# mpkuse/cerebro

Measured on AMD Instinct MI355X. Metric: loop-queries/sec (ticks of 3 descriptors vs 4096-D x 1M DB), higher is better.
Workload: dtype f64

## Files before the change

cerebro_amd/capi.py:

```python
from __future__ import annotations

import ctypes as C
import os
import sys
from pathlib import Path

import numpy as np

_HERE = Path(__file__).resolve().parent
PRODUCT_LIB_PATH = _HERE / "lib" / "libcerebro_hip.so"
HOOKS_LIB_PATH = _HERE / "lib" / "hooks" / "libcerebro_hip.so"


def _lib_path() -> Path:
    override = os.environ.get("CHIP_LIB")
    if override:
        if os.environ.get("CHIP_ALLOW_LIB_OVERRIDE") == "1":
            return Path(override).resolve()
        sys.stderr.write(f"[cerebro_amd] CHIP_LIB={override} IGNORED: set CHIP_ALLOW_LIB_OVERRIDE=1 to load another build of the library\n")
    return PRODUCT_LIB_PATH


LIB_PATH = _lib_path()

# ... 164 lines not shown
    "chip_loop_tick_enqueue": (C.c_int, [_P, C.c_int64, C.POINTER(DotParams), C.c_int32]),
    "chip_loop_tick_collect": (C.c_int, [_P, C.c_int32, C.POINTER(TickResult)]),
    "chip_loop_last_l": (C.c_int64, [_P]),
    "chip_loop_reset": (None, [_P]),
    "chip_scan_local": (C.c_int, [_P, C.c_int64, C.POINTER(DotParams), C.c_int32, _P, C.POINTER(C.c_int32)]),
    "chip_merge_decide": (C.c_int, [_P, C.c_int64, C.POINTER(DotParams), _P, C.c_int32, C.c_int32, C.POINTER(TickResult)]),
    "chip_merge_decide_enqueue": (C.c_int, [_P, C.c_int64, C.POINTER(DotParams), _P, C.c_int32, C.c_int32, C.c_int32]),
    "chip_debug_merge_lists": (C.c_int, [_P, C.c_int32, _P, C.c_int32, C.c_int32, C.c_int32, _P, C.c_int64, C.POINTER(DotParams),
                                         C.POINTER(TickResult)]),
    "chip_ransac_params_default": (None, [C.POINTER(RansacParams)]),
    "chip_pnp_ransac": (C.c_int, [_P, _P, _P, C.c_int32, C.POINTER(RansacParams), _P, C.POINTER(C.c_float), _P,
                                  C.POINTER(RansacSummary)]),
    "chip_pnp_ransac_batch": (C.c_int, [_P, C.c_int32, _P, _P, _P, C.POINTER(RansacParams), _P, _P, _P, _P, _P]),
    "chip_icp_params_default": (None, [C.POINTER(RansacParams)]),
    "chip_icp_ransac": (C.c_int, [_P, _P, _P, C.c_int32, C.POINTER(RansacParams), _P, C.POINTER(C.c_float), _P,
                                  C.POINTER(RansacSummary)]),
    "chip_icp_ransac_enqueue": (C.c_int, [_P, _P, _P, C.c_int32, C.POINTER(RansacParams)]),
    "chip_icp_ransac_collect": (C.c_int, [_P, _P, C.POINTER(C.c_float), _P, C.POINTER(RansacSummary)]),
    "chip_build_has_icp_batch": (C.c_int, []),
    "chip_icp_ransac_batch": (C.c_int, [_P, C.c_int32, _P, _P, _P, C.POINTER(RansacParams), _P, _P, _P, _P, _P]),
    "chip_debug_ransac_record": (C.c_int, [_P, C.c_int32, C.c_int32, C.POINTER(RansacShape), _P, _P, _P, _P, _P, _P, _P]),
    "chip_debug_pnp_stage": (C.c_int, [_P, C.c_int32, _P, _P, _P]),
    "chip_debug_pnp_keep_stage": (C.c_int, [_P, C.c_int32]),
    "chip_build_has_match": (C.c_int, []),
    "chip_build_has_tick_coalesce": (C.c_int, []),
    "chip_debug_coalesce_stats": (C.c_int, [_P, C.POINTER(C.c_int64), C.POINTER(C.c_int64)]),
    "chip_debug_coalesce_force": (C.c_int, [_P, C.c_int32]),
    "chip_debug_coalesce_decide": (C.c_int, [C.c_int32, C.c_int32, C.c_int32]),
    "chip_debug_last_scan": (C.c_int, [_P, C.POINTER(ScanLaunch)]),
    "chip_debug_scan_plan": (C.c_int, [C.c_int32, C.c_int32, C.c_int32, C.c_int32, C.c_int64, C.c_int32, C.c_int32, C.POINTER(ScanLaunch)]),
    "chip_debug_multi_plan": (C.c_int, [C.c_int32, C.c_int32, C.c_int32, C.c_int32, C.c_int32, C.POINTER(ScanLaunch)]),
    "chip_debug_prefilter_plan": (C.c_int, [C.c_int32, C.c_int32, C.c_int32, C.c_int32, C.POINTER(ScanLaunch)]),
    "chip_debug_prefilter_stats": (C.c_int, [_P, C.POINTER(C.c_int64), C.POINTER(C.c_int64), C.POINTER(C.c_int64)]),
    "chip_orb_match": (C.c_int, [_P, _P, C.c_int32, _P, C.c_int32, _P, _P]),
    "chip_gms_filter": (C.c_int, [_P, _P, C.c_int32, C.c_int32, C.c_int32, _P, C.c_int32, C.c_int32, C.c_int32, _P, _P, C.c_int32, _P,
                                  C.POINTER(C.c_int32)]),
    "chip_match_pair": (C.c_int, [_P, C.POINTER(MatchFrame), C.POINTER(MatchFrame), _P, C.POINTER(MatchSummary)]),
    "chip_match_read_sets": (C.c_int, [_P, C.POINTER(MatchSetsOut)]),
    "chip_pnp_ransac_matched": (C.c_int, [_P, C.c_int32, C.POINTER(RansacParams), _P, C.POINTER(C.c_float), _P, C.POINTER(RansacSummary)]),
    "chip_icp_ransac_matched": (C.c_int, [_P, C.POINTER(RansacParams), _P, C.POINTER(C.c_float), _P, C.POINTER(RansacSummary)]),
    "chip_build_has_gms_modes": (C.c_int, []),
    "chip_gms_filter_modes": (C.c_int, [_P, _P, C.c_int32, C.c_int32, C.c_int32, _P, C.c_int32, C.c_int32, C.c_int32, _P, _P, C.c_int32,
                                        C.c_uint32, _P, C.POINTER(C.c_int32), C.POINTER(GmsChoice)]),
    "chip_match_batch_modes": (C.c_int, [_P, C.POINTER(MatchFrame), C.POINTER(MatchFrame), C.c_int32, _P, C.c_uint32, C.POINTER(MatchSummary),
                                         C.POINTER(GmsChoice)]),
    "chip_match_batch_stored_modes": (C.c_int, [_P, C.c_int64, _P, C.c_int32, _P, C.c_uint32, C.POINTER(MatchSummary), C.POINTER(GmsChoice)]),
    "chip_build_has_match_batch": (C.c_int, []),
    "chip_match_batch": (C.c_int, [_P, C.POINTER(MatchFrame), C.POINTER(MatchFrame), C.c_int32, _P, C.POINTER(MatchSummary)]),
    "chip_match_select": (C.c_int, [_P, C.c_int32]),
    "chip_match_batch_read_matches": (C.c_int, [_P, C.c_int32, _P, _P]),
    "chip_pnp_ransac_matched_batch": (C.c_int, [_P, C.c_int32, _P, _P, C.POINTER(RansacParams), _P, _P, _P, _P, _P, _P]),
    "chip_icp_ransac_matched_batch_enqueue": (C.c_int, [_P, C.c_int32, _P, C.POINTER(RansacParams), _P, _P]),
    "chip_icp_ransac_matched_batch_collect": (C.c_int, [_P, _P, _P, _P, _P]),
    "chip_icp_ransac_matched_batch": (C.c_int, [_P, C.c_int32, _P, C.POINTER(RansacParams), _P, _P, _P, _P, _P, _P]),
    "chip_build_has_frame_store": (C.c_int, []),
    "chip_frame_store_reserve": (C.c_int, [_P, C.c_int32, C.c_int32]),
    "chip_frame_store_info": (C.c_int, [_P, C.POINTER(C.c_int32), C.POINTER(C.c_int32), C.POINTER(C.c_int32)]),
    "chip_frame_put": (C.c_int, [_P, C.c_int64, C.POINTER(MatchFrame)]),
    "chip_frame_drop": (C.c_int, [_P, C.c_int64]),
    "chip_frame_read": (C.c_int, [_P, C.c_int64, C.POINTER(C.c_int32), C.POINTER(C.c_int32), C.POINTER(C.c_int32), _P, _P, _P]),
    "chip_match_batch_stored": (C.c_int, [_P, C.c_int64, _P, C.c_int32, _P, C.POINTER(MatchSummary)]),
    "chip_build_has_match_pairs": (C.c_int, []),
    "chip_match_pairs_stored": (C.c_int, [_P, _P, _P, C.c_int32, _P, C.c_uint32, C.POINTER(MatchSummary), C.POINTER(GmsChoice)]),
    "chip_get_info": (C.c_int, [_P, C.POINTER(Info)]),
    "chip_profile_enable": (C.c_int, [_P, C.c_int32]),
    "chip_profile_reset": (C.c_int, [_P]),
# ... 271 lines not shown
        return r

    def resident_pause(self):
        self._chk(self.lib.chip_resident_pause(self.h), "chip_resident_pause")

    def resident_resume(self):
        self._chk(self.lib.chip_resident_resume(self.h), "chip_resident_resume")

    def loop_tick_enqueue(self, l: int, slot: int, params: DotParams | None = None):
        p = params or default_dot_params()
        self._chk(self.lib.chip_loop_tick_enqueue(self.h, l, C.byref(p), slot), "chip_loop_tick_enqueue")

    def loop_tick_collect(self, slot: int) -> TickResult:
        r = TickResult()
        self._chk(self.lib.chip_loop_tick_collect(self.h, slot, C.byref(r)), "chip_loop_tick_collect")
        return r

    def loop_reset(self):
        self.lib.chip_loop_reset(self.h)

    def last_l(self) -> int:
        return int(self.lib.chip_loop_last_l(self.h))

    def coalesce_stats(self) -> tuple[int, int]:
        passes, ticks = C.c_int64(), C.c_int64()
        self._chk(self.lib.chip_debug_coalesce_stats(self.h, C.byref(passes), C.byref(ticks)), "chip_debug_coalesce_stats")
        return passes.value, ticks.value

    def prefilter_stats(self) -> tuple[int, int, int]:
        passes, ticks, unc = C.c_int64(), C.c_int64(), C.c_int64()
        self._chk(self.lib.chip_debug_prefilter_stats(self.h, C.byref(passes), C.byref(ticks), C.byref(unc)), "chip_debug_prefilter_stats")
        return passes.value, ticks.value, unc.value

    def coalesce_force(self, on: bool):
        self._chk(self.lib.chip_debug_coalesce_force(self.h, 1 if on else 0), "chip_debug_coalesce_force")

    def last_scan(self) -> dict:
        out = ScanLaunch()
        self._chk(self.lib.chip_debug_last_scan(self.h, C.byref(out)), "chip_debug_last_scan")
        return out.as_dict()

    def scan_local(self, l: int, dev_out_ptr: int, topk: int = CHIP_DEFAULT_TOPK, params: DotParams | None = None) -> int:
        p = params or default_dot_params()
        status = C.c_int32()
        self._chk(self.lib.chip_scan_local(self.h, l, C.byref(p), topk, C.c_void_p(dev_out_ptr), C.byref(status)),
                  "chip_scan_local")
        return status.value

    def merge_decide(self, l: int, dev_gathered_ptr: int, n_lists: int, topk: int = CHIP_DEFAULT_TOPK,
                     params: DotParams | None = None) -> TickResult:
        p = params or default_dot_params()
        r = TickResult()
        self._chk(self.lib.chip_merge_decide(self.h, l, C.byref(p), C.c_void_p(dev_gathered_ptr), n_lists, topk,
                                             C.byref(r)), "chip_merge_decide")
        return r

    def merge_decide_enqueue(self, l: int, dev_gathered_ptr: int, n_lists: int, slot: int, topk: int = CHIP_DEFAULT_TOPK,
                             params: DotParams | None = None):
        p = params or default_dot_params()
        self._chk(self.lib.chip_merge_decide_enqueue(self.h, l, C.byref(p), C.c_void_p(dev_gathered_ptr), n_lists, topk, slot),
                  "chip_merge_decide_enqueue")

    def debug_merge_lists(self, form: int, scores: np.ndarray, idx: np.ndarray, l: int = 0, params: DotParams | None = None,
                          record: bool = False):
        scores = np.ascontiguousarray(scores, dtype=np.float64)
        idx = np.ascontiguousarray(idx, dtype=np.int64)
# ... 399 lines not shown
```

cerebro_amd/csrc/chip_api.hip:

```cpp
#include "chip_internal.h"
#include <cmath>
#include <cstdlib>
#include <cstring>
#include <memory>
#include <new>

using namespace chip;

extern "C" {

const char *chip_strerror(int status)
{
    switch (status) {
        case CHIP_OK: return "ok";
        case CHIP_ERR_INVALID_ARG: return "invalid argument";
        case CHIP_ERR_NO_DEVICE: return "no usable HIP device";
        case CHIP_ERR_HIP: return "HIP runtime error (see chip_last_hip_error)";
        case CHIP_ERR_OOM: return "out of device memory";
        case CHIP_ERR_NOT_F32: return "descriptor value not exactly representable as float32";
        case CHIP_ERR_NONFINITE: return "NaN/Inf in descriptor";
        case CHIP_ERR_RANGE: return "index / length out of range";
        case CHIP_ERR_UNSUPPORTED: return "unsupported configuration";
        case CHIP_ERR_TOO_FEW_POINTS: return "fewer than 20 correspondences";
        case CHIP_ERR_BUSY: return "async slot busy or empty";
// ... 176 lines not shown
    int rc = c->seg_table_dev.alloc(c, kMaxSegs);
    if (rc == CHIP_OK) rc = configure_storage(c, elem);
    if (rc != CHIP_OK) return rc;
    c->stage_bytes = 64ull << 20;
    if (c->stage_bytes < (size_t)c->D * 8 * 64) c->stage_bytes = (size_t)c->D * 8 * 64;
    rc = c->stage_dev.alloc(c, c->stage_bytes);
    if (rc == CHIP_OK) rc = c->flags_dev.alloc(c, 1);
    if (rc == CHIP_OK) rc = c->flags_host.alloc(c, 1);
    if (rc == CHIP_OK) rc = c->norm2_dev.alloc(c, 1);
    if (rc == CHIP_OK) rc = c->norm2_host.alloc(c, 1);
    if (rc != CHIP_OK) return rc;
    CHIP_HIP(c, hipMemset(c->norm2_dev, 0, sizeof(unsigned long long)));
    *c->norm2_host.host() = 0;

    scan_read_knobs(c);
    CHIP_HIP(c, hipStreamCreateWithFlags(&c->s_scan, hipStreamNonBlocking));
    {
        const int ns = c->scan_streams;
        if (ns >= 2) CHIP_HIP(c, hipStreamCreateWithFlags(&c->s_scan2, hipStreamNonBlocking));
        for (int i = 0; i < 2; i++)
            if (ns >= 3 + i) CHIP_HIP(c, hipStreamCreateWithFlags(&c->s_scan_x[i], hipStreamNonBlocking));
    }
    for (int i = 0; i < Ctx::kRing; i++) {
        constexpr size_t kListsPerGroup = 3 * kPrefilterTicks > CHIP_MAX_NQ ? 3 * kPrefilterTicks : CHIP_MAX_NQ;
        static_assert(kPrefilterTicks >= kMultiMaxTicks, "the list buffers are sized for the deepest pass");
        rc = c->partial_dev[i].alloc(c, ((size_t)c->max_grid + 1) * kListsPerGroup * CHIP_MAX_TOPK);
        if (rc != CHIP_OK) return rc;
        CHIP_HIP(c, hipEventCreateWithFlags(&c->ev_scan[i], hipEventDisableTiming));
        CHIP_HIP(c, hipEventCreateWithFlags(&c->ev_merged[i], hipEventDisableTiming));
    }
    rc = c->tickets_dev.alloc(c, Ctx::kRing);
    if (rc != CHIP_OK) return rc;
    CHIP_HIP(c, hipMemset(c->tickets_dev, 0, Ctx::kRing * sizeof(int32_t)));
    c->coalesce_max = env_int("CHIP_TICK_COALESCE", kPrefilterTicks);
    if (c->coalesce_max < 2) c->coalesce_max = 0;
    if (c->coalesce_max > kPrefilterTicks) c->coalesce_max = kPrefilterTicks;
    c->tick_poll = env_int("CHIP_TICK_POLL", 1) != 0;
    resident_read_knobs(c);
    rc = c->seq_all.alloc(c, CHIP_MAX_INFLIGHT);
    if (rc != CHIP_OK) return rc;
    std::memset(c->seq_all.host(), 0, sizeof(unsigned long long) * CHIP_MAX_INFLIGHT);
    rc = c->cert_all.alloc(c, CHIP_MAX_INFLIGHT * 4);
    if (rc != CHIP_OK) return rc;
    std::memset(c->cert_all.host(), 0, sizeof(uint32_t) * CHIP_MAX_INFLIGHT * 4);
    rc = c->topk.alloc(c, (size_t)CHIP_MAX_NQ * CHIP_MAX_TOPK);
    if (rc != CHIP_OK) return rc;
    for (Slot &s : c->slots) {
        CHIP_HIP(c, hipEventCreateWithFlags(&s.done, hipEventDisableTiming));
        rc = s.rec.alloc(c, 1);
        if (rc != CHIP_OK) return rc;
        s.seq_host = c->seq_all.host() + (&s - c->slots);
        s.seq_dev = c->seq_all.dev() + (&s - c->slots);
        s.cert_host = c->cert_all.host() + 4 * (&s - c->slots);
        s.cert_dev = c->cert_all.dev() + 4 * (&s - c->slots);
    }
    if (env_int("CHIP_SCAN_STAMPS", 0)) {
        rc = c->stamps_dev.alloc(c, (size_t)c->max_grid * 16 * 4 + 64);
        if (rc != CHIP_OK) return rc;
        CHIP_HIP(c, hipMemset(c->stamps_dev, 0, ((size_t)c->max_grid * 16 * 4 + 64) * sizeof(unsigned long long)));
    }
    rc = pnp_create(c);
    if (rc != CHIP_OK) return rc;
    c->cap_hint = capacity_hint;
    if (capacity_hint > 0) {
        std::lock_guard<std::mutex> lk(c->append_mu);
        rc = ensure_capacity(c, local_count(c, capacity_hint));
// ... 207 lines not shown
}

int64_t published_rows(const Ctx *c)
{
    std::lock_guard<std::mutex> lk(c->mu);
    return c->rows_global;
}

int tick_begin(Slot &s, int64_t n_rows, int64_t *last_l, int64_t l, const chip_dot_params *p, int32_t *status, int64_t *k)
{
    if (s.state != SlotState::Free) return CHIP_ERR_BUSY;
    const int rc = tick_prepare(n_rows, *last_l, l, p, status, k);
    if (rc != CHIP_OK) return rc;
    s.prev_last_l = *last_l;
    s.prefilter = false;
    s.tick_l = l;
    s.last_l_ptr = last_l;
    if (*status != CHIP_TICK_SCANNED) {
        if (*status == CHIP_TICK_TOO_SHORT) *last_l = l;
        fill_immediate(s.rec.host(), *status);
        s.state = SlotState::Immediate;
    }
    return CHIP_OK;
}

static int tick_submit(Ctx *c, int64_t k, int64_t l, const chip_dot_params *p, const void *const *q, bool sync_tick, Slot &s)
{
    ScanRequest rq;
    rq.k = k; rq.q = q; rq.nq = 3; rq.K = CHIP_DEFAULT_TOPK;
    rq.res = s.rec.dev(); rq.l = l; rq.p = p;
    rq.tick = true; rq.sync_tick = sync_tick; rq.merge_on_scan_stream = true;
    if (c->tick_poll) { s.seq_want = ++c->tick_seq; rq.seq_dev = s.seq_dev; rq.seq_val = s.seq_want; }
    ScanReceipt done;
    const int rc = enqueue_scan_merge(c, rq, &done);
    if (rc != CHIP_OK) return rc;
    if (done.done_ev) s.wait_ev = done.done_ev;
    else { CHIP_HIP(c, hipEventRecord(s.done, done.merge_stream)); s.wait_ev = s.done; }
    s.pass_no = c->pass_no;
    s.state = c->tick_poll && done.fused ? SlotState::Poll : SlotState::Event;
    return CHIP_OK;
}

int coalesce_decide(int n_parked, int t_max, bool scan_running)
{
    if (t_max < 2) return kCoalesceLaunch;
    if (!scan_running) return n_parked > 0 ? kCoalesceParkFlush : kCoalesceLaunch;
    return n_parked + 1 >= t_max ? kCoalesceParkFlush : kCoalescePark;
}

static int coalesce_ticks_max(const Ctx *c, int64_t k, bool sync_tick)
{
    if (c->coalesce_max < 2 || sync_tick || c->nranks != 1 || c->xchg || c->parent || c->group || !c->own_query_stream) return 0;
    if ((double)k * c->D * c->elem <= c->scan_overlap_bytes) return 0;
    int fit = scan_multi_max_ticks(c);
    if (c->coalesce_max >= kPrefilterTicks && scan_prefilter_usable(c)) fit = kPrefilterTicks;
    const int t = fit < c->coalesce_max ? fit : c->coalesce_max;
    return t >= 2 ? t : 0;
}

static int coalesce_submit(Ctx *c, int T)
{
    const int b = (int)(c->n_enqueued++ % Ctx::kRing);
    const int K = CHIP_DEFAULT_TOPK;
    const bool prefilter = T == kPrefilterTicks;
    static_assert(kPrefilterTicks > kMultiMaxTicks, "a pass of kPrefilterTicks ticks is the prefilter's");
    PassArgs a{};
    scan_args_db(c, &a);
    a.K = K;
    a.partial = c->partial_dev[b];
    for (int t = 0; t < T; t++) {
        a.k[t] = c->parked[t].k;
        if (a.k[t] > a.n_rows) a.n_rows = a.k[t];
        for (int i = 0; i < 3; i++) a.q[3 * t + i] = c->parked[t].q[i];
    }
    const int grid = scan_multi_grid(c);
    double E = 0.0;
    if (prefilter) {
        std::lock_guard<std::mutex> lk(c->mu);
        E = prefilter_error_bound(c->D, c->row_norm_max);
    }
    if (hipEventQuery(c->ev_merged[b]) != hipSuccess) CHIP_HIP(c, hipStreamWaitEvent(c->s_scan, c->ev_merged[b], 0));
    hipEvent_t e1 = nullptr;
    int rc = c->prof_on ? prof_begin(c, c->s_scan, (double)a.n_rows * c->D * c->elem, &e1) : CHIP_OK;
    if (rc == CHIP_OK) rc = prefilter ? launch_scan_prefilter(c, c->s_scan, a, grid) : launch_scan_multi(c, c->s_scan, a, T, grid);
    if (rc != CHIP_OK) return rc;
    if (e1) CHIP_HIP(c, hipEventRecord(e1, c->s_scan));
    CHIP_HIP(c, hipEventRecord(c->ev_scan[b], c->s_scan));
    c->pass_ev = c->ev_scan[b];
    c->pass_no++;
    CHIP_HIP(c, hipStreamWaitEvent(c->s_query, c->ev_scan[b], 0));
    chip_topk_entry *exact = c->partial_dev[b] + (size_t)kPrefilterTicks * grid * 3 * K;
    if (prefilter) {
        RescoreArgs ra{};
        ra.seg_table = a.seg_table; ra.seg_shift = a.seg_shift; ra.seg_mask = a.seg_mask; ra.D = a.D; ra.K = K;
        ra.in = c->partial_dev[b]; ra.n_lists = grid; ra.wpb = 8;
        ra.E = E;
        ra.out = exact;
        for (int t = 0; t < T; t++) {
            const Ctx::ParkedTick &pt = c->parked[t];
            Slot &s = *pt.slot;
            ra.k[t] = pt.k;
            for (int i = 0; i < 3; i++) { ra.q[3 * t + i] = s.pf_q[i] = pt.q[i]; s.cert_host[i] = 0; }
            ra.cert[t] = s.cert_dev;
            s.prefilter = true; s.pf_k = pt.k; s.pf_p = pt.p;
        }
        rc = launch_rescore(c, c->s_query, ra);
        if (rc != CHIP_OK) return rc;
    }
    for (int t = 0; t < T; t++) {
        const Ctx::ParkedTick &pt = c->parked[t];
        if (prefilter) rc = launch_merge(c, c->s_query, merge_args(exact + (size_t)t * 3 * K, 1, K, nullptr, pt.slot->rec.dev(), pt.l, &pt.p), 3);
        else rc = launch_merge(c, c->s_query, merge_args(c->partial_dev[b] + (size_t)t * grid * 3 * K, grid, K, nullptr, pt.slot->rec.dev(), pt.l, &pt.p), 3);
        if (rc != CHIP_OK) return rc;
        CHIP_HIP(c, hipEventRecord(pt.slot->done, c->s_query));
        pt.slot->wait_ev = pt.slot->done;
        pt.slot->state = SlotState::Event;
        pt.slot->pass_no = c->pass_no;
    }
    CHIP_HIP(c, hipEventRecord(c->ev_merged[b], c->s_query));
    c->coalesce_passes++;
    c->coalesce_ticks += T;
    if (prefilter) { c->prefilter_passes++; c->prefilter_ticks += T; }
    return CHIP_OK;
}

int coalesce_flush(Ctx *c)
{
    const int T = c->n_parked;
    if (T == 0) return CHIP_OK;
    c->n_parked = 0;
    const Ctx::ParkedTick &p0 = c->parked[0];
    int rc;
    if (T == kPrefilterTicks && !scan_prefilter_usable(c)) {
        const Ctx::ParkedTick &pl = c->parked[T - 1];
        rc = coalesce_submit(c, T - 1);
        if (rc == CHIP_OK) rc = tick_submit(c, pl.k, pl.l, &pl.p, pl.q, false, *pl.slot);
    } else {
        rc = T == 1 ? tick_submit(c, p0.k, p0.l, &p0.p, p0.q, false, *p0.slot) : coalesce_submit(c, T);
    }
    for (int t = 0; t < T && rc != CHIP_OK; t++) {
        c->parked[t].slot->state = SlotState::Failed;
        c->parked[t].slot->err = rc;
    }
    return rc;
}

static int tick_enqueue_slot(Ctx *c, int64_t l, const chip_dot_params *p, bool sync_tick, Slot &s)
{
    int32_t status = 0;
    int64_t k = 0;
    const int64_t n_pub = published_rows(c);
    int rc = tick_begin(s, c->xchg ? INT64_MAX : n_pub, &c->last_l, l, p, &status, &k);
// ... 670 lines not shown
    info->capacity_local = (int64_t)r->segs.size() * r->seg_rows;
    info->lossy_rows = r->lossy_rows;
    std::strncpy(info->arch, r->arch, sizeof(info->arch) - 1);
    info->storage_bytes = r->elem;
    info->n_devices = c->group ? group_size(c) : 1;
    info->exchange = c->group ? c->group_transport : (c->xchg ? CHIP_EXCHANGE_RCCL : CHIP_EXCHANGE_NONE);
    info->comm_ranks = exchange_comm_ranks(c->group ? r : c);
    info->comm_init_abandoned = c->comm_init_abandoned;
    info->scan_forms = scan_forms_built();
    info->test_hooks = chip_build_test_hooks();
    info->row_norm_max = r->row_norm_max;
    return CHIP_OK;
}

int chip_debug_coalesce_stats(chip_ctx *c, int64_t *passes, int64_t *ticks)
{
    if (!c || !passes || !ticks || c->group) return CHIP_ERR_INVALID_ARG;
    std::lock_guard<std::mutex> qlk(c->query_mu);
    *passes = c->coalesce_passes;
    *ticks = c->coalesce_ticks;
    return CHIP_OK;
}

int chip_debug_prefilter_stats(chip_ctx *c, int64_t *passes, int64_t *ticks, int64_t *uncertified)
{
    if (!c || !passes || !ticks || !uncertified || c->group) return CHIP_ERR_INVALID_ARG;
    std::lock_guard<std::mutex> qlk(c->query_mu);
    *passes = c->prefilter_passes;
    *ticks = c->prefilter_ticks;
    *uncertified = c->prefilter_uncertified;
    return CHIP_OK;
}

int chip_debug_coalesce_force(chip_ctx *c, int32_t on)
{
    if (!c || c->group) return CHIP_ERR_INVALID_ARG;
    std::lock_guard<std::mutex> qlk(c->query_mu);
    c->coalesce_force = on != 0;
    if (!on) { (void)hipSetDevice(c->device); (void)coalesce_flush(c); }
    return CHIP_OK;
}

int chip_debug_coalesce_decide(int32_t n_parked, int32_t t_max, int32_t scan_running) { return coalesce_decide(n_parked, t_max, scan_running != 0); }

int chip_debug_last_scan(chip_ctx *c, chip_debug_scan_launch *out)
{
    if (!c || !out || c->group) return CHIP_ERR_INVALID_ARG;
    std::lock_guard<std::mutex> qlk(c->query_mu);
    (void)hipSetDevice(c->device);
    (void)coalesce_flush(c);
    *out = c->last_scan;
    return CHIP_OK;
}

int chip_debug_scan_plan(int32_t D, int32_t elem, int32_t nq, int32_t K, int64_t n_rows, int32_t call, int32_t n_cus, chip_debug_scan_launch *out)
{
    if (!out || D <= 0 || (elem != 4 && elem != 8) || nq < 1 || nq > CHIP_MAX_NQ || K < 1 || K > CHIP_MAX_TOPK || n_rows < 0 || n_cus < 1 ||
        call < CHIP_SCAN_CALL_QUERY || call > CHIP_SCAN_CALL_TICK_SYNC)
        return CHIP_ERR_INVALID_ARG;
    if (D % 4 != 0 || (size_t)D * 4 * CHIP_MAX_NQ > 160 * 1024 || (elem == 8 && (size_t)D * 8 * 2 > 160 * 1024)) return CHIP_ERR_UNSUPPORTED;
    std::unique_ptr<Ctx> c(new (std::nothrow) Ctx());
    if (!c) return CHIP_ERR_OOM;
    c->D = D;
    c->elem = elem;
    c->n_cus = n_cus;
    scan_read_knobs(c.get());
// ... 93 lines not shown
```

cerebro_amd/csrc/chip_internal.h:

```cpp
#pragma once
#include <hip/hip_runtime.h>
#include <cstdint>
#include <mutex>
#include <condition_variable>
#include <vector>
#include "../../include/cerebro_hip.h"

namespace chip {

constexpr int kWave = 64;
constexpr int kMaxSegs = 4096;
constexpr int64_t kSegBytesTarget = 512ll << 20;

struct ScanArgs {
    const void *const *seg_table;
    int32_t seg_shift;
    int64_t seg_mask;
    int64_t n_rows;
    int32_t D;
    int32_t K;
    const void *q[CHIP_MAX_NQ];
    int64_t idx_mul, idx_add;
    chip_topk_entry *partial;
    int32_t q64 = 0;
// ... 35 lines not shown
    uint32_t done;
    uint32_t direct;
};

constexpr int kMultiMaxTicks = 3;
constexpr int kPrefilterTicks = 4;
constexpr int kRescoreCap = 32;
struct PassArgs {
    const void *const *seg_table;
    int32_t seg_shift;
    int64_t seg_mask;
    int64_t n_rows;
    int32_t D;
    int32_t K;
    int64_t k[kPrefilterTicks];
    const void *q[3 * kPrefilterTicks];
    chip_topk_entry *partial;
};
struct RescoreArgs {
    const void *const *seg_table;
    int32_t seg_shift;
    int64_t seg_mask;
    int32_t D;
    int32_t K;
    const chip_topk_entry *in;
    int32_t n_lists;
    int32_t wpb;
    int64_t k[kPrefilterTicks];
    const void *q[3 * kPrefilterTicks];
    double E;
    chip_topk_entry *out;
    uint32_t *cert[kPrefilterTicks];
};

struct MergeArgs {
    const chip_topk_entry *in;
    int32_t n_lists;
    int32_t K;
    chip_topk_entry *out;
    chip_tick_result *result;
    int64_t l;
    int32_t locality;
    double thresh;
};

struct Ctx;

template <class T> class DevBuf {
public:
    DevBuf() = default;
    DevBuf(const DevBuf &) = delete;
    DevBuf &operator=(const DevBuf &) = delete;
    ~DevBuf() { release(); }
    int alloc(Ctx *c, size_t n);
    int reserve(Ctx *c, size_t n);
    void release() { if (p_) (void)hipFree(p_); p_ = nullptr; cap_ = 0; }
    T *get() const { return p_; }
    operator T *() const { return p_; }
    size_t capacity() const { return cap_; }
private:
    T *p_ = nullptr;
    size_t cap_ = 0;
};
template <class T> class PinnedBuf {
public:
    PinnedBuf() = default;
    PinnedBuf(const PinnedBuf &) = delete;
    PinnedBuf &operator=(const PinnedBuf &) = delete;
    ~PinnedBuf() { release(); }
    int alloc(Ctx *c, size_t n);
    int reserve(Ctx *c, size_t n);
    void release() { if (h_) (void)hipHostFree(h_); h_ = d_ = nullptr; cap_ = 0; }
    T *host() const { return h_; }
    T *dev() const { return d_; }
    size_t capacity() const { return cap_; }
private:
    T *h_ = nullptr, *d_ = nullptr;
    size_t cap_ = 0;
};

int launch_resident(Ctx *c, hipStream_t s, const ResidentArgs &ra, int grid);
int launch_scan(Ctx *c, hipStream_t s, const ScanArgs &a, int nq, int grid);
int launch_merge(Ctx *c, hipStream_t s, const MergeArgs &a, int nq);
int scan_multi_max_ticks(const Ctx *c);
int scan_multi_plan(int D, int elem, int n_ticks, int K, int grid, chip_debug_scan_launch *f);
int scan_multi_grid(const Ctx *c);
int launch_scan_multi(Ctx *c, hipStream_t s, const PassArgs &a, int n_ticks, int grid);
int scan_prefilter_plan(int D, int elem, int K, int grid, chip_debug_scan_launch *f);
bool scan_prefilter_usable(const Ctx *c);
double prefilter_error_bound(int D, double row_norm_max);
int launch_scan_prefilter(Ctx *c, hipStream_t s, const PassArgs &a, int grid);
int launch_rescore(Ctx *c, hipStream_t s, const RescoreArgs &a);
int scan_grid_for(const Ctx *c, int64_t n_rows, int nq, bool q64);
bool scan_q64(const Ctx *c, int nq, bool long_scan);
int scan_rows_form(const Ctx *c, int64_t n_rows, int nq, int grid, bool q64, bool sync_tick = false);
int scan_select(const Ctx *c, const ScanArgs &a, int nq, int grid, chip_debug_scan_launch *f);
int scan_forms_built();
int launch_scores(Ctx *c, hipStream_t s, const ScanArgs &a, double *out_dev);
int launch_store_rows(Ctx *c, hipStream_t s, const void *src, int src_elem, int64_t n, int64_t first_global, uint32_t *flags_dev, bool write_ring,
                      int64_t row_stride = 1);
int launch_synth(Ctx *c, hipStream_t s, int64_t first_global, int64_t n, uint64_t seed,
                 const int64_t *plant_dst_dev, const int64_t *plant_src_dev, const int32_t *plant_kind_dev, int64_t n_plant, int unit);

enum class SlotState : uint8_t {
    Free,
    Immediate,
    Parked,
    Event,
    Poll,
    Resident,
    Failed,
};

struct Slot {
    hipEvent_t done = nullptr;
    hipEvent_t wait_ev = nullptr;
    PinnedBuf<chip_tick_result> rec;
    SlotState state = SlotState::Free;
    int64_t prev_last_l = 0;
    int64_t tick_l = 0;
    unsigned long long *seq_host = nullptr, *seq_dev = nullptr;
    unsigned long long seq_want = 0;
    uint64_t pass_no = 0;
    int32_t err = 0;
    bool prefilter = false;
// ... 92 lines not shown
    PinnedBuf<unsigned long long> seq_all;
    unsigned long long tick_seq = 0;
    bool tick_poll = true;
    bool tick_fused = true;
    Resident res;
    uint64_t n_enqueued = 0;
    int32_t max_grid = 0;
    PinnedBuf<chip_topk_entry> topk;

    DevBuf<char> qvec_dev;
    DevBuf<double> scores_dev;
    DevBuf<unsigned long long> stamps_dev;

    std::vector<char> qconv;
    int64_t cap_hint = 0;
    int32_t group_transport = 0;
    mutable int last_comm = 0;
    int32_t comm_init_abandoned = 0;
    Exchange *xchg = nullptr;
    Group *group = nullptr;
    Ctx *parent = nullptr;
    Slot slots[CHIP_MAX_INFLIGHT];
    int64_t last_l = 0;

    struct ParkedTick { Slot *slot; int64_t k, l; chip_dot_params p; const void *q[3]; };
    int32_t coalesce_max = 4;
    bool coalesce_force = false;
    ParkedTick parked[kPrefilterTicks];
    int32_t n_parked = 0;
    hipEvent_t pass_ev = nullptr;
    uint64_t pass_no = 0;
    int64_t coalesce_passes = 0, coalesce_ticks = 0;
    int64_t prefilter_passes = 0, prefilter_ticks = 0, prefilter_uncertified = 0;
    PinnedBuf<uint32_t> cert_all;
    chip_debug_scan_launch last_scan{};

    int32_t scan_block = 0;
    int32_t scan_blocks_per_cu = 2;
    int32_t scan_reserve = 0;
    int32_t scan_variant = 0;
    int32_t scan_streams = 4;
    bool tick_same_stream = true;
    int32_t scan_claim = -1;
    int32_t scan_rows = 0;
    double scan_plain_bytes = 768.0 * 1024 * 1024;
    double scan_sync_plain_bytes = 4096.0 * 1024 * 1024;
    double scan_half_bytes = 192.0 * 1024 * 1024;
    int32_t scan_short_bpc = 1;
    double scan_overlap_bytes = 8.0 * 1024 * 1024 * 1024;

    bool prof_on = false;
    std::vector<hipEvent_t> prof_ev;
    size_t prof_used = 0;
    double prof_bytes_last = 0.0;

    PnpState *pnp_state = nullptr;
    IcpState *icp_state = nullptr;
    BatchState *batch_state = nullptr;
    MatchState *match_state = nullptr;
    std::mutex match_mu;

    mutable hipError_t last_hip = hipSuccess;
};

#define CHIP_HIP(ctx, expr)                                  \
    do {                                                     \
// ... 182 lines not shown
```

cerebro_amd/csrc/kernels.hip:

```cpp
#include "chip_internal.h"
#include "topk_merge.h"
#include <cmath>
#include <type_traits>

namespace chip {

typedef float f32x4 __attribute__((ext_vector_type(4)));
typedef double f64x2 __attribute__((ext_vector_type(2)));

template <typename T> struct Vec16;
template <> struct Vec16<float> { typedef f32x4 type; static constexpr int N = 4; };
template <> struct Vec16<double> { typedef f64x2 type; static constexpr int N = 2; };

template <typename V>
__device__ __forceinline__ const __attribute__((address_space(1))) V *as_global(const V *p)
{
    return (const __attribute__((address_space(1))) V *)p;
}

template <typename V>
__device__ __forceinline__ V stream_load(const V *p)
{
    return __builtin_nontemporal_load(as_global(p));
}
// ... 624 lines not shown
                slot_wait<L - R - 1 - g>();
                static_for<R>([&](auto rr) CHIP_INLINE_LAMBDA { prefilter_fma_slot<pass_row_slot(u, rr), QR>(acc[rr][NS + g]); });
                static_for<R>([&](auto rr) CHIP_INLINE_LAMBDA { prefilter_fma_slot<pass_row_slot(u, rr) + 2, QR + 2>(acc[rr][NS + g]); });
            });
            slots_issue_kib<u, NG>(voff, row, qg);
        });
    }
};

template <int NG>
__global__ __launch_bounds__(kMultiBlock) __attribute__((amdgpu_num_vgpr(pass_vgpr_base(kPrefilterMaxNG) / 2))) void db_scan_prefilter(PassArgs a)
{
    static_assert(NG <= kPrefilterMaxNG, "the compiler's share is sized for kPrefilterMaxNG query slots per KiB");
    shared_pass<PassF32<NG>>(a);
}

__device__ __forceinline__ void block_best(double &bs, int64_t &bi, double *red_s, int64_t *red_i, int lane, int wave)
{
#pragma unroll
    for (int m = 32; m >= 1; m >>= 1) {
        const double os = __shfl_xor(bs, m, 64);
        const int64_t oi = __shfl_xor(bi, m, 64);
        if (key_gt(os, oi, bs, bi)) { bs = os; bi = oi; }
    }
    __syncthreads();
    if (lane == 0) { red_s[wave] = bs; red_i[wave] = bi; }
    __syncthreads();
    bs = red_s[0]; bi = red_i[0];
#pragma unroll
    for (int w = 1; w < 8; w++)
        if (key_gt(red_s[w], red_i[w], bs, bi)) { bs = red_s[w]; bi = red_i[w]; }
}

__global__ __launch_bounds__(512) void tick_rescore(RescoreArgs a)
{
    constexpr int MAXH = 512 * CHIP_MAX_TOPK / 512;
    __shared__ double red_s[8];
    __shared__ int64_t red_i[8];
    __shared__ chip_topk_entry cand[kRescoreCap];
    __shared__ int n_cand;
    const int tid = threadIdx.x, lane = tid & 63;
    const int wave = __builtin_amdgcn_readfirstlane(tid >> 6);
    const int tick = blockIdx.x / 3, q = blockIdx.x % 3;
    const int K = a.K, n = a.n_lists * K;
    const chip_topk_entry *in = a.in + (int64_t)tick * a.n_lists * 3 * K;
    const int64_t k = a.k[tick];
    if (tid == 0) n_cand = 0;
    double es[MAXH];
    int64_t ei[MAXH];
#pragma unroll
    for (int h = 0; h < MAXH; h++) {
        const int c = tid + 512 * h;
        es[h] = -INFINITY; ei[h] = -1;
        if (c < n) { const chip_topk_entry t = in[((int64_t)(c / K) * 3 + q) * K + (c % K)]; es[h] = t.score; ei[h] = t.idx; }
    }
    double ms = -INFINITY;
    int64_t mi = -1;
    const int64_t tw = (int64_t)a.n_lists * a.wpb;
#pragma unroll
    for (int h = 0; h < MAXH; h++) {
        const int c = tid + 512 * h;
        if (c % K != K - 1 || ei[h] < 0) continue;
        int64_t part = k % tw - (int64_t)(c / K) * a.wpb;
        part = part < 0 ? 0 : part > a.wpb ? a.wpb : part;
        if ((k / tw) * a.wpb + part > K && es[h] > ms) { ms = es[h]; mi = 0; }
    }
    block_best(ms, mi, red_s, red_i, lane, wave);
    double gs = INFINITY;
    int64_t gi = INT64_MAX;
    for (int j = 0; j < K; j++) {
        double bs = -INFINITY;
        int64_t bi = -1;
#pragma unroll
        for (int h = 0; h < MAXH; h++)
            if (key_gt(gs, gi, es[h], ei[h]) && key_gt(es[h], ei[h], bs, bi)) { bs = es[h]; bi = ei[h]; }
        block_best(bs, bi, red_s, red_i, lane, wave);
// ... 3 lines not shown
    thr -= fabs(thr) * 0x1p-51;
    const bool ok = mi < 0 || ms < thr;
#pragma unroll
    for (int h = 0; h < MAXH; h++)
        if (ei[h] >= 0 && es[h] >= thr) {
            const int at = atomicAdd(&n_cand, 1);
            if (at < kRescoreCap) { chip_topk_entry t; t.score = es[h]; t.idx = ei[h]; cand[at] = t; }
        }
    __syncthreads();
    const int nc = n_cand < kRescoreCap ? n_cand : kRescoreCap;
    const float *qrow = static_cast<const float *>(a.q[3 * tick + q]);
    for (int j = wave; j < nc; j += 8) {
        const int64_t r = cand[j].idx;
        const float *row[1] = {static_cast<const float *>(a.seg_table[r >> a.seg_shift]) + (r & a.seg_mask) * (int64_t)a.D};
        double acc[1][1];
        rows_dot<float, 1, 4, true, 1, 1>(row, qrow, a.D, lane, acc);
        const double s = butterfly_sum(acc[0][0]);
        if (lane == 0) cand[j].score = s;
    }
    __syncthreads();
    if (wave == 0) {
        static_assert(kRescoreCap <= 64, "one lane per candidate");
        chip_topk_entry *out = a.out + (int64_t)(3 * tick + q) * K;
        chip_topk_entry me;
        me.score = -INFINITY; me.idx = -1;
        if (lane < nc) me = cand[lane];
        int rank = 0;
        for (int j = 0; j < nc; j++) {
            const chip_topk_entry o = cand[j];
            rank += key_gt(o.score, o.idx, me.score, me.idx) ? 1 : 0;
        }
        if (lane < nc && rank < K) out[rank] = me;
        if (lane >= nc && lane < K) out[lane] = me;
        if (lane == 0) a.cert[tick][q] = ok && n_cand <= kRescoreCap ? 1u : 2u;
    }
}

template <int NQ, int NG, bool FULL>
__global__ __launch_bounds__(1024) void db_scan_topk_wide(ScanArgs a)
{
    static_assert(NG >= 1 && NG < NQ, "at least one query staged, at least one read in place");
    extern __shared__ __attribute__((aligned(16))) char smem[];
    double *qs = reinterpret_cast<double *>(smem);
    constexpr int NL = NQ - NG, U = 4, CH = 128;
    const int D = a.D, K = a.K;
    const int tid = threadIdx.x, lane = tid & 63;
    const int wave = __builtin_amdgcn_readfirstlane(tid >> 6);
    const int wpb = blockDim.x >> 6;
    stage_queries<double, NL>(a, qs, tid, blockDim.x);
    __syncthreads();
    const double *qg[NG];
#pragma unroll
    for (int g = 0; g < NG; g++) qg[g] = static_cast<const double *>(a.q[NL + g]);

    double my_s[NQ], thr_s[NQ];
    int64_t my_i[NQ], thr_i[NQ];
#pragma unroll
    for (int q = 0; q < NQ; q++) { my_s[q] = -INFINITY; my_i[q] = -1; thr_s[q] = -INFINITY; thr_i[q] = -1; }
    const int e0 = lane * 2;
    const int64_t tw = (int64_t)gridDim.x * wpb;
    for (int64_t r = (int64_t)blockIdx.x * wpb + wave; r < a.n_rows; r += tw) {
        const double *row = row_base<double>(a, r);
        double acc[NQ];
#pragma unroll
        for (int q = 0; q < NQ; q++) acc[q] = 0.0;
        for (int base = 0; base < D; base += CH * U) {
            f64x2 v[U];
// ... 859 lines not shown
}

template <class Kernel>
static int launch_pass(Ctx *c, hipStream_t s, Kernel kernel, const PassArgs &a, chip_debug_scan_launch f)
{
    CHIP_HIP(c, hipFuncSetAttribute(reinterpret_cast<const void *>(kernel), hipFuncAttributeMaxDynamicSharedMemorySize, f.lds_bytes));
    hipLaunchKernelGGL(kernel, dim3(f.grid), dim3(kMultiBlock), f.lds_bytes, s, a);
    CHIP_HIP(c, hipGetLastError());
    f.n_rows = a.n_rows;
    f.launches = c->last_scan.launches + 1;
    c->last_scan = f;
    return CHIP_OK;
}

int launch_scan_multi(Ctx *c, hipStream_t s, const PassArgs &a, int n_ticks, int grid)
{
    chip_debug_scan_launch f;
    if (n_ticks > scan_multi_max_ticks(c) || grid > c->max_grid || scan_multi_plan(c->D, c->elem, n_ticks, a.K, grid, &f) != CHIP_OK)
        return CHIP_ERR_UNSUPPORTED;
    if (c->elem == 4) return n_ticks == 2 ? launch_pass(c, s, db_scan_topk_multi<2>, a, f) : launch_pass(c, s, db_scan_topk_multi<3>, a, f);
    static_assert(kSharedF64MaxTicks == 2 && kSharedMaxNG == 2, "the instantiations below");
    if (f.NG == 0) return launch_pass(c, s, db_scan_shared_f64<2, 0>, a, f);
    if (f.NG == 1) return launch_pass(c, s, db_scan_shared_f64<2, 1>, a, f);
    return launch_pass(c, s, db_scan_shared_f64<2, 2>, a, f);
}

int launch_scan_prefilter(Ctx *c, hipStream_t s, const PassArgs &a, int grid)
{
    chip_debug_scan_launch f;
    if (grid > c->max_grid || scan_prefilter_plan(c->D, c->elem, a.K, grid, &f) != CHIP_OK) return CHIP_ERR_UNSUPPORTED;
    return f.NG == 0 ? launch_pass(c, s, db_scan_prefilter<0>, a, f) : launch_pass(c, s, db_scan_prefilter<kPrefilterMaxNG>, a, f);
}

int launch_rescore(Ctx *c, hipStream_t s, const RescoreArgs &a)
{
    if (a.n_lists > 512 || a.K > CHIP_MAX_TOPK) return CHIP_ERR_UNSUPPORTED;
    hipLaunchKernelGGL(tick_rescore, dim3(3 * kPrefilterTicks), dim3(512), 0, s, a);
    CHIP_HIP(c, hipGetLastError());
    return CHIP_OK;
}

int launch_resident(Ctx *c, hipStream_t s, const ResidentArgs &ra, int grid)
{
#ifdef CHIP_NO_ROWS_FORM
    (void)c; (void)s; (void)ra; (void)grid;
    return CHIP_ERR_UNSUPPORTED;
#else
    int block, bpc;
    scan_shape(c, 3, false, &block, &bpc);
    const size_t lds = scan_lds_bytes(c, 3, 1, block, false, true);
    if (lds + 64 > 160 * 1024 || grid > 512) return CHIP_ERR_UNSUPPORTED;
    return c->elem == 8 ? launch_resident_T<double>(c, s, ra, grid, lds, block) : launch_resident_T<float>(c, s, ra, grid, lds, block);
#endif
}

template <typename T, bool FULL>
__global__ __launch_bounds__(512) void db_scan_scores(ScanArgs a, double *out)
{
    extern __shared__ __attribute__((aligned(16))) char smem[];
    T *qs = reinterpret_cast<T *>(smem);
    const int tid = threadIdx.x, lane = tid & 63;
    const int wave = __builtin_amdgcn_readfirstlane(tid >> 6);
    const int wpb = blockDim.x >> 6;
    stage_queries<T, 1>(a, qs, tid, blockDim.x);
    __syncthreads();
    const int64_t tw = (int64_t)gridDim.x * wpb;
    for (int64_t r = (int64_t)blockIdx.x * wpb + wave; r < a.n_rows; r += tw) {
        const T *row[1] = {row_base<T>(a, r)};
        double acc[1][1];
        rows_dot<T, 1, 4, FULL, FULL ? 6 : 1, 1>(row, qs, a.D, lane, acc);
// ... 310 lines not shown
```

include/cerebro_hip.h:

```cpp
#ifndef CEREBRO_HIP_H
#define CEREBRO_HIP_H
#include <stdint.h>

#ifdef __cplusplus
extern "C" {
#endif

#define CHIP_ABI_VERSION 7

enum {
    CHIP_OK = 0,
    CHIP_ERR_INVALID_ARG = -1,
    CHIP_ERR_NO_DEVICE = -2,
    CHIP_ERR_HIP = -3,
    CHIP_ERR_OOM = -4,
    CHIP_ERR_NOT_F32 = -5,
    CHIP_ERR_NONFINITE = -6,
    CHIP_ERR_RANGE = -7,
    CHIP_ERR_UNSUPPORTED = -8,
    CHIP_ERR_TOO_FEW_POINTS = -9,
    CHIP_ERR_BUSY = -10,
    CHIP_ERR_COMM = -11,
    CHIP_ERR_SHARD_FAILED = -12,
    CHIP_ERR_GROUP_BROKEN = -13
// ... 93 lines not shown

#define CHIP_SCAN_FAMILY_NONE    0
#define CHIP_SCAN_FAMILY_ONE_ROW 1
#define CHIP_SCAN_FAMILY_WIDE    2
#define CHIP_SCAN_FAMILY_ROWS    3
#define CHIP_SCAN_FAMILY_MULTI   4
#define CHIP_SCAN_FAMILY_PREFILTER 5
#define CHIP_SCAN_CALL_QUERY      0
#define CHIP_SCAN_CALL_TICK       1
#define CHIP_SCAN_CALL_TICK_SYNC  2
typedef struct {
    int32_t family;
    int32_t elem;
    int32_t nq, K;
    int32_t U, NT, FULL;
    int32_t NG;
    int32_t R, NTL;
    int32_t ticks;
    int32_t q64;
    int32_t claimed;
    int32_t fused;
    int32_t grid, block;
    int32_t wg_per_cu;
    int32_t lds_bytes;
    int64_t n_rows;
    int64_t launches;
} chip_debug_scan_launch;
int chip_debug_last_scan(chip_ctx *ctx, chip_debug_scan_launch *out);
int chip_debug_scan_plan(int32_t D, int32_t elem, int32_t nq, int32_t K, int64_t n_rows, int32_t call, int32_t n_cus,
                         chip_debug_scan_launch *out);
int chip_debug_multi_plan(int32_t D, int32_t elem, int32_t n_ticks, int32_t K, int32_t n_cus, chip_debug_scan_launch *out);
int chip_debug_prefilter_plan(int32_t D, int32_t elem, int32_t K, int32_t n_cus, chip_debug_scan_launch *out);
int chip_debug_prefilter_stats(chip_ctx *ctx, int64_t *passes, int64_t *ticks, int64_t *uncertified);

typedef struct { double score; int64_t idx; } chip_topk_entry;
int chip_scan_local(chip_ctx *ctx, int64_t l, const chip_dot_params *p, int32_t topk, void *dev_out, int32_t *status);
int chip_merge_decide(chip_ctx *ctx, int64_t l, const chip_dot_params *p, const void *dev_gathered, int32_t n_lists,
                      int32_t topk, chip_tick_result *out);
int chip_merge_decide_enqueue(chip_ctx *ctx, int64_t l, const chip_dot_params *p, const void *dev_gathered, int32_t n_lists,
                              int32_t topk, int32_t slot);
int chip_debug_merge_lists(chip_ctx *ctx, int32_t form, const chip_topk_entry *lists, int32_t n_lists, int32_t nq, int32_t K,
                           chip_topk_entry *out, int64_t l, const chip_dot_params *p, chip_tick_result *result);

typedef struct {
    double  error_thresh;
    double  min_inlier_ratio;
    int32_t max_iterations;
    int32_t min_iterations;
    int32_t use_mle;
    int32_t sample_size;
    double  failure_probability;
    uint64_t seed;
    int32_t n_hypotheses;
    int32_t sampler;
} chip_ransac_params;
enum { CHIP_SAMPLER_FRESH = 0, CHIP_SAMPLER_THEIA_PERSISTENT = 1 };
void chip_ransac_params_default(chip_ransac_params *p);

typedef struct {
    int32_t n_iterations;
    int32_t n_inliers;
    int32_t best_hypothesis;
    int32_t n_models;
    double  best_cost;
} chip_ransac_summary;

// ... 166 lines not shown
```

Measured before the change: 1227.

## Fuse prefilter rescore and per-tick merges into one pass-finish kernel

Replaces the separate rescore kernel and the per-tick merge launches with a single pass_finish kernel. In that kernel the last of the three query blocks per tick, chosen through an atomic ticket counter, performs the merge and writes the certificate. It also records one event per pass instead of one per tick and lets slots use polling when tick_poll is enabled. This cuts kernel launch and event overhead on the coalesced tick path, at the cost of device-side atomics and a last-block-done pattern. It also adds a debug histogram of pass sizes.

```diff
diff --git a/cerebro_amd/capi.py b/cerebro_amd/capi.py
--- a/cerebro_amd/capi.py
+++ b/cerebro_amd/capi.py
@@ -220,6 +220,7 @@
     "chip_debug_multi_plan": (C.c_int, [C.c_int32, C.c_int32, C.c_int32, C.c_int32, C.c_int32, C.POINTER(ScanLaunch)]),
     "chip_debug_prefilter_plan": (C.c_int, [C.c_int32, C.c_int32, C.c_int32, C.c_int32, C.POINTER(ScanLaunch)]),
     "chip_debug_prefilter_stats": (C.c_int, [_P, C.POINTER(C.c_int64), C.POINTER(C.c_int64), C.POINTER(C.c_int64)]),
+    "chip_debug_coalesce_hist": (C.c_int, [_P, C.POINTER(C.c_int64)]),
     "chip_orb_match": (C.c_int, [_P, _P, C.c_int32, _P, C.c_int32, _P, _P]),
     "chip_gms_filter": (C.c_int, [_P, _P, C.c_int32, C.c_int32, C.c_int32, _P, C.c_int32, C.c_int32, C.c_int32, _P, _P, C.c_int32, _P,
                                   C.POINTER(C.c_int32)]),
@@ -557,6 +558,11 @@
         self._chk(self.lib.chip_debug_prefilter_stats(self.h, C.byref(passes), C.byref(ticks), C.byref(unc)), "chip_debug_prefilter_stats")
         return passes.value, ticks.value, unc.value
 
+    def coalesce_hist(self) -> list[int]:
+        out = (C.c_int64 * 5)()
+        self._chk(self.lib.chip_debug_coalesce_hist(self.h, out), "chip_debug_coalesce_hist")
+        return list(out)
+
     def coalesce_force(self, on: bool):
         self._chk(self.lib.chip_debug_coalesce_force(self.h, 1 if on else 0), "chip_debug_coalesce_force")
 
diff --git a/cerebro_amd/csrc/chip_api.hip b/cerebro_amd/csrc/chip_api.hip
--- a/cerebro_amd/csrc/chip_api.hip
+++ b/cerebro_amd/csrc/chip_api.hip
@@ -232,6 +232,9 @@
     rc = c->tickets_dev.alloc(c, Ctx::kRing);
     if (rc != CHIP_OK) return rc;
     CHIP_HIP(c, hipMemset(c->tickets_dev, 0, Ctx::kRing * sizeof(int32_t)));
+    rc = c->finish_tickets.alloc(c, (size_t)Ctx::kRing * kPrefilterTicks);
+    if (rc != CHIP_OK) return rc;
+    CHIP_HIP(c, hipMemset(c->finish_tickets, 0, (size_t)Ctx::kRing * kPrefilterTicks * sizeof(uint32_t)));
     c->coalesce_max = env_int("CHIP_TICK_COALESCE", kPrefilterTicks);
     if (c->coalesce_max < 2) c->coalesce_max = 0;
     if (c->coalesce_max > kPrefilterTicks) c->coalesce_max = kPrefilterTicks;
@@ -505,8 +508,10 @@
     rq.tick = true; rq.sync_tick = sync_tick; rq.merge_on_scan_stream = true;
     if (c->tick_poll) { s.seq_want = ++c->tick_seq; rq.seq_dev = s.seq_dev; rq.seq_val = s.seq_want; }
     ScanReceipt done;
+    const uint64_t passes = c->pass_no;
     const int rc = enqueue_scan_merge(c, rq, &done);
     if (rc != CHIP_OK) return rc;
+    if (c->pass_no != passes) c->pass_hist[1]++;
     if (done.done_ev) s.wait_ev = done.done_ev;
     else { CHIP_HIP(c, hipEventRecord(s.done, done.merge_stream)); s.wait_ev = s.done; }
     s.pass_no = c->pass_no;
@@ -562,35 +567,38 @@
     c->pass_ev = c->ev_scan[b];
     c->pass_no++;
     CHIP_HIP(c, hipStreamWaitEvent(c->s_query, c->ev_scan[b], 0));
-    chip_topk_entry *exact = c->partial_dev[b] + (size_t)kPrefilterTicks * grid * 3 * K;
+    FinishArgs fa{};
+    RescoreArgs &ra = fa.r;
+    ra.K = K;
+    ra.in = c->partial_dev[b]; ra.n_lists = grid;
     if (prefilter) {
-        RescoreArgs ra{};
-        ra.seg_table = a.seg_table; ra.seg_shift = a.seg_shift; ra.seg_mask = a.seg_mask; ra.D = a.D; ra.K = K;
-        ra.in = c->partial_dev[b]; ra.n_lists = grid; ra.wpb = 8;
+        ra.seg_table = a.seg_table; ra.seg_shift = a.seg_shift; ra.seg_mask = a.seg_mask; ra.D = a.D;
+        ra.wpb = 8;
         ra.E = E;
-        ra.out = exact;
-        for (int t = 0; t < T; t++) {
-            const Ctx::ParkedTick &pt = c->parked[t];
-            Slot &s = *pt.slot;
-            ra.k[t] = pt.k;
-            for (int i = 0; i < 3; i++) { ra.q[3 * t + i] = s.pf_q[i] = pt.q[i]; s.cert_host[i] = 0; }
-            ra.cert[t] = s.cert_dev;
-            s.prefilter = true; s.pf_k = pt.k; s.pf_p = pt.p;
-        }
-        rc = launch_rescore(c, c->s_query, ra);
-        if (rc != CHIP_OK) return rc;
+        ra.out = c->partial_dev[b] + (size_t)kPrefilterTicks * grid * 3 * K;
+        fa.ticket = c->finish_tickets + (size_t)b * kPrefilterTicks;
     }
     for (int t = 0; t < T; t++) {
         const Ctx::ParkedTick &pt = c->parked[t];
-        if (prefilter) rc = launch_merge(c, c->s_query, merge_args(exact + (size_t)t * 3 * K, 1, K, nullptr, pt.slot->rec.dev(), pt.l, &pt.p), 3);
-        else rc = launch_merge(c, c->s_query, merge_args(c->partial_dev[b] + (size_t)t * grid * 3 * K, grid, K, nullptr, pt.slot->rec.dev(), pt.l, &pt.p), 3);
-        if (rc != CHIP_OK) return rc;
-        CHIP_HIP(c, hipEventRecord(pt.slot->done, c->s_query));
-        pt.slot->wait_ev = pt.slot->done;
-        pt.slot->state = SlotState::Event;
-        pt.slot->pass_no = c->pass_no;
-    }
+        Slot &s = *pt.slot;
+        fa.rec[t] = s.rec.dev(); fa.l[t] = pt.l; fa.locality[t] = pt.p.locality; fa.thresh[t] = pt.p.thresh;
+        if (c->tick_poll) { s.seq_want = ++c->tick_seq; fa.seq[t] = s.seq_dev; fa.seq_val[t] = s.seq_want; }
+        if (!prefilter) continue;
+        ra.k[t] = pt.k;
+        for (int i = 0; i < 3; i++) { ra.q[3 * t + i] = s.pf_q[i] = pt.q[i]; s.cert_host[i] = 0; }
+        ra.cert[t] = s.cert_dev;
+        s.prefilter = true; s.pf_k = pt.k; s.pf_p = pt.p;
+    }
+    rc = launch_pass_finish(c, c->s_query, fa, T, prefilter);
+    if (rc != CHIP_OK) return rc;
     CHIP_HIP(c, hipEventRecord(c->ev_merged[b], c->s_query));
+    for (int t = 0; t < T; t++) {
+        Slot &s = *c->parked[t].slot;
+        s.wait_ev = c->ev_merged[b];
+        s.state = c->tick_poll ? SlotState::Poll : SlotState::Event;
+        s.pass_no = c->pass_no;
+    }
+    c->pass_hist[T]++;
     c->coalesce_passes++;
     c->coalesce_ticks += T;
     if (prefilter) { c->prefilter_passes++; c->prefilter_ticks += T; }
@@ -1327,6 +1335,16 @@
     return CHIP_OK;
 }
 
+int chip_debug_coalesce_hist(chip_ctx *c, int64_t out[5])
+{
+    static_assert(kPrefilterTicks == 4, "out[5] of the header");
+    if (!c || !out || c->group) return CHIP_ERR_INVALID_ARG;
+    std::lock_guard<std::mutex> qlk(c->query_mu);
+    out[0] = 0;
+    for (int t = 1; t <= kPrefilterTicks; t++) out[t] = c->pass_hist[t];
+    return CHIP_OK;
+}
+
 int chip_debug_coalesce_force(chip_ctx *c, int32_t on)
 {
     if (!c || c->group) return CHIP_ERR_INVALID_ARG;
diff --git a/cerebro_amd/csrc/chip_internal.h b/cerebro_amd/csrc/chip_internal.h
--- a/cerebro_amd/csrc/chip_internal.h
+++ b/cerebro_amd/csrc/chip_internal.h
@@ -91,6 +91,16 @@
     chip_topk_entry *out;
     uint32_t *cert[kPrefilterTicks];
 };
+struct FinishArgs {
+    RescoreArgs r;
+    chip_tick_result *rec[kPrefilterTicks];
+    int64_t l[kPrefilterTicks];
+    double thresh[kPrefilterTicks];
+    int32_t locality[kPrefilterTicks];
+    unsigned long long *seq[kPrefilterTicks];
+    unsigned long long seq_val[kPrefilterTicks];
+    uint32_t *ticket;
+};
 
 struct MergeArgs {
     const chip_topk_entry *in;
@@ -149,7 +159,7 @@
 bool scan_prefilter_usable(const Ctx *c);
 double prefilter_error_bound(int D, double row_norm_max);
 int launch_scan_prefilter(Ctx *c, hipStream_t s, const PassArgs &a, int grid);
-int launch_rescore(Ctx *c, hipStream_t s, const RescoreArgs &a);
+int launch_pass_finish(Ctx *c, hipStream_t s, const FinishArgs &a, int n_ticks, bool prefilter);
 int scan_grid_for(const Ctx *c, int64_t n_rows, int nq, bool q64);
 bool scan_q64(const Ctx *c, int nq, bool long_scan);
 int scan_rows_form(const Ctx *c, int64_t n_rows, int nq, int grid, bool q64, bool sync_tick = false);
@@ -308,6 +318,8 @@
     uint64_t pass_no = 0;
     int64_t coalesce_passes = 0, coalesce_ticks = 0;
     int64_t prefilter_passes = 0, prefilter_ticks = 0, prefilter_uncertified = 0;
+    int64_t pass_hist[kPrefilterTicks + 1] = {};
+    DevBuf<uint32_t> finish_tickets;
     PinnedBuf<uint32_t> cert_all;
     chip_debug_scan_launch last_scan{};
 
diff --git a/cerebro_amd/csrc/kernels.hip b/cerebro_amd/csrc/kernels.hip
--- a/cerebro_amd/csrc/kernels.hip
+++ b/cerebro_amd/csrc/kernels.hip
@@ -680,7 +680,7 @@
         if (key_gt(red_s[w], red_i[w], bs, bi)) { bs = red_s[w]; bi = red_i[w]; }
 }
 
-__global__ __launch_bounds__(512) void tick_rescore(RescoreArgs a)
+__device__ __forceinline__ uint32_t rescore_query(const RescoreArgs &a, int tick, int q)
 {
     constexpr int MAXH = 512 * CHIP_MAX_TOPK / 512;
     __shared__ double red_s[8];
@@ -689,7 +689,6 @@
     __shared__ int n_cand;
     const int tid = threadIdx.x, lane = tid & 63;
     const int wave = __builtin_amdgcn_readfirstlane(tid >> 6);
-    const int tick = blockIdx.x / 3, q = blockIdx.x % 3;
     const int K = a.K, n = a.n_lists * K;
     const chip_topk_entry *in = a.in + (int64_t)tick * a.n_lists * 3 * K;
     const int64_t k = a.k[tick];
@@ -759,7 +758,53 @@
         }
         if (lane < nc && rank < K) out[rank] = me;
         if (lane >= nc && lane < K) out[lane] = me;
-        if (lane == 0) a.cert[tick][q] = ok && n_cand <= kRescoreCap ? 1u : 2u;
+    }
+    return ok && n_cand <= kRescoreCap ? 1u : 2u;
+}
+
+__global__ __launch_bounds__(512) void tick_rescore(RescoreArgs a)
+{
+    const int tick = blockIdx.x / 3, q = blockIdx.x % 3;
+    const uint32_t cert = rescore_query(a, tick, q);
+    if (threadIdx.x == 0) a.cert[tick][q] = cert;
+}
+
+template <bool PREFILTER>
+__global__ __launch_bounds__(512) void pass_finish(FinishArgs a)
+{
+    __shared__ __attribute__((aligned(16))) char smem[kMergeSmem];
+    __shared__ uint32_t taken;
+    const int tick = PREFILTER ? blockIdx.x / 3 : blockIdx.x;
+    uint32_t certs = 0;
+    const chip_topk_entry *lists;
+    int n_lists;
+    if constexpr (PREFILTER) {
+        const int q = blockIdx.x % 3;
+        const uint32_t cert = rescore_query(a.r, tick, q);
+        __threadfence();
+        __syncthreads();
+        if (threadIdx.x == 0) {
+            const uint32_t mine = 1u + (cert == 1u ? 0u : 0x100u << q);
+            taken = __hip_atomic_fetch_add(a.ticket + tick, mine, __ATOMIC_RELAXED, __HIP_MEMORY_SCOPE_AGENT) + mine;
+        }
+        __syncthreads();
+        certs = taken;
+        if ((certs & 0xffu) != 3u) return;
+        __threadfence();
+        lists = a.r.out + (int64_t)tick * 3 * a.r.K;
+        n_lists = 1;
+    } else {
+        lists = a.r.in + (int64_t)tick * a.r.n_lists * 3 * a.r.K;
+        n_lists = a.r.n_lists;
+    }
+    if (PREFILTER && threadIdx.x == 0) {
+#pragma unroll
+        for (int q = 0; q < 3; q++) a.r.cert[tick][q] = (certs >> (8 + q)) & 1u ? 2u : 1u;
+    }
+    merge_sorted_lists<3>(lists, n_lists, 3, 0, a.r.K, nullptr, a.rec[tick], a.l[tick], a.locality[tick], a.thresh[tick], smem);
+    if (threadIdx.x == 0) {
+        if (PREFILTER) __hip_atomic_store(a.ticket + tick, 0u, __ATOMIC_RELAXED, __HIP_MEMORY_SCOPE_AGENT);
+        if (a.seq[tick]) __hip_atomic_store(a.seq[tick], a.seq_val[tick], __ATOMIC_RELEASE, __HIP_MEMORY_SCOPE_SYSTEM);
     }
 }
 
@@ -1685,10 +1730,11 @@
     return f.NG == 0 ? launch_pass(c, s, db_scan_prefilter<0>, a, f) : launch_pass(c, s, db_scan_prefilter<kPrefilterMaxNG>, a, f);
 }
 
-int launch_rescore(Ctx *c, hipStream_t s, const RescoreArgs &a)
-{
-    if (a.n_lists > 512 || a.K > CHIP_MAX_TOPK) return CHIP_ERR_UNSUPPORTED;
-    hipLaunchKernelGGL(tick_rescore, dim3(3 * kPrefilterTicks), dim3(512), 0, s, a);
+int launch_pass_finish(Ctx *c, hipStream_t s, const FinishArgs &a, int n_ticks, bool prefilter)
+{
+    if (a.r.n_lists > 512 || a.r.K > CHIP_MAX_TOPK || n_ticks < 1 || n_ticks > kPrefilterTicks || (prefilter && n_ticks != kPrefilterTicks)) return CHIP_ERR_UNSUPPORTED;
+    if (prefilter) hipLaunchKernelGGL(pass_finish<true>, dim3(3 * n_ticks), dim3(512), 0, s, a);
+    else hipLaunchKernelGGL(pass_finish<false>, dim3(n_ticks), dim3(512), 0, s, a);
     CHIP_HIP(c, hipGetLastError());
     return CHIP_OK;
 }
diff --git a/include/cerebro_hip.h b/include/cerebro_hip.h
--- a/include/cerebro_hip.h
+++ b/include/cerebro_hip.h
@@ -149,6 +149,7 @@
 int chip_debug_multi_plan(int32_t D, int32_t elem, int32_t n_ticks, int32_t K, int32_t n_cus, chip_debug_scan_launch *out);
 int chip_debug_prefilter_plan(int32_t D, int32_t elem, int32_t K, int32_t n_cus, chip_debug_scan_launch *out);
 int chip_debug_prefilter_stats(chip_ctx *ctx, int64_t *passes, int64_t *ticks, int64_t *uncertified);
+int chip_debug_coalesce_hist(chip_ctx *ctx, int64_t out[5]);
 
 typedef struct { double score; int64_t idx; } chip_topk_entry;
 int chip_scan_local(chip_ctx *ctx, int64_t l, const chip_dot_params *p, int32_t topk, void *dev_out, int32_t *status);
```

Result: no change. 1228 (median of 3 runs) (+0.1%).
